# y-scope/pinot

Hardware: AMD Instinct MI355X
Metric: scanned rows/sec + achieved HBM GB/s, filtered SUM on 1B-row segment (higher is better)
Workload: dtype int64

## Files before the change

### pinot_amd/csrc/pg_scan_simple_dma.h

```cpp
#pragma once
#include "pg_scan_simple.h"

namespace pg {

typedef const __attribute__((address_space(3))) uint32_t* LdsWords;

constexpr int kDmaRecordBytes = 1024;
static_assert(sizeof(BlockPartial) * (kBlockThreads / 64) + 16 <= kDmaRecordBytes, "the records and the flag fit their area");
__host__ __device__ constexpr int dma_slot_bytes(int filter_bits, int value_bits) { return 256 * (filter_bits + value_bits); }
__host__ __device__ constexpr size_t dma_lds_bytes(int filter_bits, int value_bits, int slots, int waves) {
  return (size_t)kDmaRecordBytes + (size_t)waves * slots * dma_slot_bytes(filter_bits, value_bits);
}

template <int J> __device__ __forceinline__ void dma_wait() { asm volatile("s_waitcnt vmcnt(%0)" :: "n"(J) : "memory"); }

template <int N, int kAux>
__device__ __forceinline__ void dma_stage_tile(const uint8_t* f_tile, const uint8_t* v_tile, int f_bytes, int v_bytes, int nf, uint8_t* slot, int lane) {
#pragma unroll
  for (int j = 0; j < N; ++j) {
    const bool is_f = j < nf;
    const int at = (is_f ? j : j - nf) * 1024, chunk = is_f ? f_bytes : v_bytes;
    const uint8_t* src = (is_f ? f_tile : v_tile) + at + lane * 16;
    uint8_t* dst = slot + (is_f ? 0 : f_bytes) + at;
    if (at + lane * 16 < chunk)
      __builtin_amdgcn_global_load_lds((const __attribute__((address_space(1))) void*)src, (__attribute__((address_space(3))) void*)dst, 16, 0, kAux);
  }
}

template <typename P>
__device__ __forceinline__ void dma_tile(const P& p, long long tile, int lane, const uint8_t* slot, unsigned long long& count, unsigned long long& sum,
                                         uint32_t& umin, uint32_t& umax) {
  const auto& L = p.nodes[0];
  const auto& ac = p.agg_cols[0];
  const LdsWords fw = (LdsWords)(const uint32_t*)slot + lane * L.bits;
  const LdsWords vw = (LdsWords)(const uint32_t*)(slot + 256 * L.bits) + lane * ac.bits;
  uint32_t m = L.lo == 0 ? simple_range_dispatch<true>(L.bits, fw, 0u, L.span) : simple_range_dispatch<false>(L.bits, fw, (uint32_t)L.lo, L.span);
  if (L.exclusive) m = ~m;
  const long long rem = (long long)p.num_docs - (tile * 2048 + lane * 32);
  m &= rem >= 32 ? 0xFFFFFFFFu : (rem <= 0 ? 0u : ((1u << (int)rem) - 1u));
  count += (unsigned)__builtin_popcount(m);
  uint32_t psum = 0, tmin = 0xFFFFFFFFu, tmax = 0u;
  unsigned long long wsum = 0;
  simple_agg_dispatch(ac.bits, vw, m, ac.need_sum != 0, ac.need_minmax != 0, psum, wsum, tmin, tmax);
  sum += wsum + psum;
  umin = tmin < umin ? tmin : umin;
  umax = tmax > umax ? tmax : umax;
}

template <int N, int S, int kAux, typename P>
__device__ __forceinline__ void scan_simple_dma_body(const P& p, uint32_t block_index, uint32_t num_blocks, uint8_t* lds) {
  static_assert(S >= 2 && N * (S - 1) <= 63, "vmcnt counts to 63");
  BlockPartial* red = reinterpret_cast<BlockPartial*>(lds);
  uint32_t* fold_flag_ptr = reinterpret_cast<uint32_t*>(lds + sizeof(BlockPartial) * (kBlockThreads / 64));
  const int lane = threadIdx.x & 63;
  const int wave_in_block = __builtin_amdgcn_readfirstlane((int)(threadIdx.x >> 6));
  const int waves_per_block = blockDim.x >> 6;
  const long long total_waves = (long long)num_blocks * waves_per_block;
  const long long num_tiles = ((long long)p.num_docs + 2047) / 2048;
  const auto& L = p.nodes[0];
  const auto& ac = p.agg_cols[0];
  const int f_bytes = 256 * L.bits, v_bytes = 256 * ac.bits, slot_bytes = f_bytes + v_bytes, nf = (L.bits + 3) >> 2;
  uint8_t* ring = lds + kDmaRecordBytes + (size_t)wave_in_block * S * slot_bytes;

  unsigned long long count = 0, sum = 0;
  uint32_t umin = 0xFFFFFFFFu, umax = 0u;
  const long long first = (long long)block_index * waves_per_block + wave_in_block;
  const long long n = first < num_tiles ? (num_tiles - first + total_waves - 1) / total_waves : 0;
#pragma unroll
  for (int k = 0; k < S - 1; ++k)
    if (k < n) dma_stage_tile<N, kAux>(L.fwd + (first + k * total_waves) * f_bytes, ac.fwd + (first + k * total_waves) * v_bytes, f_bytes, v_bytes, nf, ring + k * slot_bytes, lane);
  long long i = 0, tile = first;
  int rd = 0, wr = S - 1;
  for (; i + (S - 1) < n; ++i, tile += total_waves) {
    asm volatile("s_waitcnt lgkmcnt(0)" ::: "memory");
    const long long ahead = tile + (S - 1) * total_waves;
    dma_stage_tile<N, kAux>(L.fwd + ahead * f_bytes, ac.fwd + ahead * v_bytes, f_bytes, v_bytes, nf, ring + wr * slot_bytes, lane);
    dma_wait<N * (S - 1)>();
    dma_tile(p, tile, lane, ring + rd * slot_bytes, count, sum, umin, umax);
    rd = rd + 1 == S ? 0 : rd + 1;
    wr = wr + 1 == S ? 0 : wr + 1;
  }
#define PG_DMA_DRAIN(R) if (S - 1 >= R && n - i == R) { dma_wait<N * (R - 1)>(); dma_tile(p, tile, lane, ring + rd * slot_bytes, count, sum, umin, umax); \
                          rd = rd + 1 == S ? 0 : rd + 1; ++i; tile += total_waves; }
  PG_DMA_DRAIN(3) PG_DMA_DRAIN(2) PG_DMA_DRAIN(1)
#undef PG_DMA_DRAIN
  static_assert(S <= 4, "PG_DMA_DRAIN covers rings of up to four slots");

  BlockPartial mine;
  partial_identity(mine);
  mine.count = (unsigned long long)wave_sum_i64((long long)count);
  mine.sum[0] = wave_sum_i64((long long)sum);
  mine.kmin[0] = wave_min_i32(umin == 0xFFFFFFFFu ? 0x7FFFFFFF : (int32_t)umin);
  mine.kmax[0] = wave_max_i32(count == 0ull ? (int32_t)0x80000000 : (int32_t)umax);
  if (lane == 0) red[wave_in_block] = mine;
  __syncthreads();
  publish_block_partial(p, red, waves_per_block, fold_flag_ptr, block_index, num_blocks);
}


}
```

Before: 1804 billion.

## Copy LDS tile into registers before restaging its slot in DMA ring

```diff
diff --git a/pinot_amd/csrc/pg_scan_simple_dma.h b/pinot_amd/csrc/pg_scan_simple_dma.h
--- a/pinot_amd/csrc/pg_scan_simple_dma.h
+++ b/pinot_amd/csrc/pg_scan_simple_dma.h
@@ -5,11 +5,16 @@
 
 typedef const __attribute__((address_space(3))) uint32_t* LdsWords;
 
+#ifndef PG_DMA_READ_GROUP
+#define PG_DMA_READ_GROUP 2
+#endif
+constexpr int kDmaReadGroup = PG_DMA_READ_GROUP;
 constexpr int kDmaRecordBytes = 1024;
+constexpr int kDmaReadPadBytes = (4 * (kDmaReadGroup - 1) + 15) / 16 * 16;
 static_assert(sizeof(BlockPartial) * (kBlockThreads / 64) + 16 <= kDmaRecordBytes, "the records and the flag fit their area");
 __host__ __device__ constexpr int dma_slot_bytes(int filter_bits, int value_bits) { return 256 * (filter_bits + value_bits); }
 __host__ __device__ constexpr size_t dma_lds_bytes(int filter_bits, int value_bits, int slots, int waves) {
-  return (size_t)kDmaRecordBytes + (size_t)waves * slots * dma_slot_bytes(filter_bits, value_bits);
+  return (size_t)kDmaRecordBytes + (size_t)waves * slots * dma_slot_bytes(filter_bits, value_bits) + kDmaReadPadBytes;
 }
 
 template <int J> __device__ __forceinline__ void dma_wait() { asm volatile("s_waitcnt vmcnt(%0)" :: "n"(J) : "memory"); }
@@ -27,24 +32,42 @@
   }
 }
 
-template <typename P>
-__device__ __forceinline__ void dma_tile(const P& p, long long tile, int lane, const uint8_t* slot, unsigned long long& count, unsigned long long& sum,
-                                         uint32_t& umin, uint32_t& umax) {
+template <typename P, typename WF, typename WV>
+__device__ __forceinline__ void dma_decode(const P& p, long long tile, int lane, WF fw, WV vw, unsigned long long& count, unsigned long long& sum,
+                                           uint32_t& umin, uint32_t& umax) {
   const auto& L = p.nodes[0];
   const auto& ac = p.agg_cols[0];
-  const LdsWords fw = (LdsWords)(const uint32_t*)slot + lane * L.bits;
-  const LdsWords vw = (LdsWords)(const uint32_t*)(slot + 256 * L.bits) + lane * ac.bits;
+#if defined(PG_DMA_DIAG) && PG_DMA_DIAG == 1
+#pragma unroll
+  for (int k = 0; k < kSimpleMaxBits; ++k) asm volatile("" :: "v"(fw[k]), "v"(vw[k]));
+  return;
+#endif
   uint32_t m = L.lo == 0 ? simple_range_dispatch<true>(L.bits, fw, 0u, L.span) : simple_range_dispatch<false>(L.bits, fw, (uint32_t)L.lo, L.span);
   if (L.exclusive) m = ~m;
   const long long rem = (long long)p.num_docs - (tile * 2048 + lane * 32);
   m &= rem >= 32 ? 0xFFFFFFFFu : (rem <= 0 ? 0u : ((1u << (int)rem) - 1u));
   count += (unsigned)__builtin_popcount(m);
+#if defined(PG_DMA_DIAG) && PG_DMA_DIAG == 2
+#pragma unroll
+  for (int k = 0; k < kSimpleMaxBits; ++k) asm volatile("" :: "v"(vw[k]));
+  return;
+#endif
   uint32_t psum = 0, tmin = 0xFFFFFFFFu, tmax = 0u;
   unsigned long long wsum = 0;
   simple_agg_dispatch(ac.bits, vw, m, ac.need_sum != 0, ac.need_minmax != 0, psum, wsum, tmin, tmax);
   sum += wsum + psum;
   umin = tmin < umin ? tmin : umin;
   umax = tmax > umax ? tmax : umax;
+}
+
+__device__ __forceinline__ void dma_read_out(LdsWords w, int bits, uint32_t (&r)[kSimpleMaxBits]) {
+  static_assert(kSimpleMaxBits % kDmaReadGroup == 0, "whole groups");
+#pragma unroll
+  for (int k = 0; k < kSimpleMaxBits; k += kDmaReadGroup)
+    if (k < bits) {
+#pragma unroll
+      for (int j = 0; j < kDmaReadGroup; ++j) r[k + j] = w[k + j];
+    }
 }
 
 template <int N, int S, int kAux, typename P>
@@ -66,25 +89,61 @@
   uint32_t umin = 0xFFFFFFFFu, umax = 0u;
   const long long first = (long long)block_index * waves_per_block + wave_in_block;
   const long long n = first < num_tiles ? (num_tiles - first + total_waves - 1) / total_waves : 0;
+  long long i = 0, tile = first;
+  int rd = 0;
+#ifndef PG_DMA_DECODE_FROM_SLOT
+  auto stage = [&](long long t, int slot) __attribute__((always_inline)) { dma_stage_tile<N, kAux>(L.fwd + t * f_bytes, ac.fwd + t * v_bytes, f_bytes, v_bytes, nf, ring + slot * slot_bytes, lane); };
+  auto tile_from_registers = [&](bool restage) __attribute__((always_inline)) {
+    uint32_t fr[kSimpleMaxBits], vr[kSimpleMaxBits];
+    const uint8_t* slot = ring + rd * slot_bytes;
+    dma_read_out((LdsWords)(const uint32_t*)slot + lane * L.bits, L.bits, fr);
+    dma_read_out((LdsWords)(const uint32_t*)(slot + f_bytes) + lane * ac.bits, ac.bits, vr);
+    asm volatile("s_waitcnt lgkmcnt(0)" ::: "memory");
+    if (restage) stage(tile + S * total_waves, rd);
+#pragma unroll
+    for (int k = 0; k < kSimpleMaxBits; ++k) asm volatile("" : "+v"(fr[k]), "+v"(vr[k]));
+    __builtin_amdgcn_sched_barrier(0);
+    dma_decode(p, tile, lane, fr, vr, count, sum, umin, umax);
+    rd = rd + 1 == S ? 0 : rd + 1;
+    ++i;
+    tile += total_waves;
+  };
+#pragma unroll
+  for (int k = 0; k < S; ++k)
+    if (k < n) stage(first + k * total_waves, k);
+  while (i + S < n) {
+    dma_wait<N * (S - 1)>();
+    tile_from_registers(true);
+  }
+#define PG_DMA_DRAIN(R) if (S >= R && n - i == R) { dma_wait<N * (R - 1)>(); tile_from_registers(false); }
+  PG_DMA_DRAIN(4) PG_DMA_DRAIN(3) PG_DMA_DRAIN(2) PG_DMA_DRAIN(1)
+#undef PG_DMA_DRAIN
+  static_assert(S <= 4, "PG_DMA_DRAIN covers rings of up to four slots");
+#else
+  auto tile_from_slot = [&]() __attribute__((always_inline)) {
+    const uint8_t* slot = ring + rd * slot_bytes;
+    dma_decode(p, tile, lane, (LdsWords)(const uint32_t*)slot + lane * L.bits, (LdsWords)(const uint32_t*)(slot + f_bytes) + lane * ac.bits, count, sum, umin, umax);
+    rd = rd + 1 == S ? 0 : rd + 1;
+    ++i;
+    tile += total_waves;
+  };
 #pragma unroll
   for (int k = 0; k < S - 1; ++k)
     if (k < n) dma_stage_tile<N, kAux>(L.fwd + (first + k * total_waves) * f_bytes, ac.fwd + (first + k * total_waves) * v_bytes, f_bytes, v_bytes, nf, ring + k * slot_bytes, lane);
-  long long i = 0, tile = first;
-  int rd = 0, wr = S - 1;
-  for (; i + (S - 1) < n; ++i, tile += total_waves) {
+  int wr = S - 1;
+  while (i + (S - 1) < n) {
     asm volatile("s_waitcnt lgkmcnt(0)" ::: "memory");
     const long long ahead = tile + (S - 1) * total_waves;
     dma_stage_tile<N, kAux>(L.fwd + ahead * f_bytes, ac.fwd + ahead * v_bytes, f_bytes, v_bytes, nf, ring + wr * slot_bytes, lane);
     dma_wait<N * (S - 1)>();
-    dma_tile(p, tile, lane, ring + rd * slot_bytes, count, sum, umin, umax);
-    rd = rd + 1 == S ? 0 : rd + 1;
+    tile_from_slot();
     wr = wr + 1 == S ? 0 : wr + 1;
   }
-#define PG_DMA_DRAIN(R) if (S - 1 >= R && n - i == R) { dma_wait<N * (R - 1)>(); dma_tile(p, tile, lane, ring + rd * slot_bytes, count, sum, umin, umax); \
-                          rd = rd + 1 == S ? 0 : rd + 1; ++i; tile += total_waves; }
+#define PG_DMA_DRAIN(R) if (S - 1 >= R && n - i == R) { dma_wait<N * (R - 1)>(); tile_from_slot(); }
   PG_DMA_DRAIN(3) PG_DMA_DRAIN(2) PG_DMA_DRAIN(1)
 #undef PG_DMA_DRAIN
   static_assert(S <= 4, "PG_DMA_DRAIN covers rings of up to four slots");
+#endif
 
   BlockPartial mine;
   partial_identity(mine);
```

After: 1785 billion. -1.0%, worse.
